# OATML-Markslab/ProteinGym

Measured on AMD Instinct MI355X. Metric: mutants scored/sec (ESM-1v 650M masked-marginal), higher is better.
Workload: dtype f16x3 (fp32 operands split into 2 fp16 planes, 3 fp16 MFMAs per product, fp32 accumulate)

## Files before the change

include/pgmi.h:

```cpp
#ifndef PGMI_H
#define PGMI_H

#include <stddef.h>
#include <stdint.h>

#ifdef __cplusplus
extern "C" {
#endif

#define PGMI_ABI_VERSION 5

#define PGMI_OK 0
#define PGMI_EINVAL (-1)
#define PGMI_ENOMEM (-2)
#define PGMI_EHIP (-3)
#define PGMI_ENODEV (-4)
#define PGMI_EPARSE (-5)
#define PGMI_EOVERFLOW (-6)

#define PGMI_ARCH_ESM1B 1
#define PGMI_ARCH_ESM2 2
#define PGMI_ARCH_TRANCEPTION 3
#define PGMI_ARCH_MSA 4
#define PGMI_ARCH_PROGEN2 5
// ... 111 lines not shown
int pgmi_op_gemm(int device, int precision, const float* A, const float* W, const float* bias,
                 const float* residual, int M, int N, int K, int epilogue ,
                 float* C);
int pgmi_op_qkln_prep(int device, const float* qkv, const float* q_w, const float* k_w, int B, int T, int H, int iters, float* qk,
                      float* v, double* ms);
int pgmi_op_attention(int device, int precision, const float* qkv, const int32_t* kv_len,
                      int B, int T, int H, int rotary, float* ctx);
int pgmi_op_causal_attention(int device, int lanes, const float* X, const float* W, const float* bias, int K, const float* qkv,
                             const float* conv, const float* rot_cos, const float* rot_sin, const float* slopes, int B, int T,
                             int heads, float* ctx);
int pgmi_op_prefix_attention(int device, const float* qkv, const int32_t* seg_off, int n_seg, const float* prefix_kv, int P, int heads,
                             int split, float* ctx);
int pgmi_op_cross_attention(int device, const float* q, const int32_t* seg_off, int n_seg, const float* mem_kv, int S, int heads,
                            int split, float* ctx);
int pgmi_op_rmsnorm(int device, const float* x, const float* w, int rows, int D, float eps, float* y);
int pgmi_op_geom_attention(int device, const float* proj, const float* rot, const float* trans, const int32_t* frame_mask,
                           int per_row_frames, const float* w_rot, const float* w_dist, int B, int S, int H, float* out);
int pgmi_op_geom_key_tile(int S);
int pgmi_op_moe(int device, const float* h, const float* gate, const float* w1, const float* w3, const float* w2, int M, int D, int F,
                int E, int top_k, int gated, float* out, int32_t* ids, float* weights);
int pgmi_op_tied_row_attention(int device, const float* qkv, int R, int C, int H, int splits, float* ctx, float* probs);
int pgmi_op_tied_row_splits(int R, int C, int H);
int pgmi_op_column_attention(int device, const float* X, const float* W, const float* bias, int K, int R, int C, int H, float* ctx);

int pgmi_tr_token_logprobs(pgmi_model* m, const int32_t* tokens, int B, int T, float* out);
int pgmi_tr_sequence_loglik(pgmi_model* m, const int32_t* tokens, const int32_t* lens, int B, int T,
                            const float* log_prior, int P, const int32_t* prior_a0, const int32_t* prior_row0,
                            const int32_t* prior_n, const int32_t* prior_flip, float alpha, float* out);
int pgmi_tr_sequence_loglik_shared(pgmi_model* m, const int32_t* tokens, const int32_t* ref, int B, int T,
                                   const float* log_prior, int P, const int32_t* prior_a0, const int32_t* prior_row0,
// ... 166 lines not shown
```

proteingym_amd/_lib.py:

```python
from __future__ import annotations

import ctypes as C
import os

import numpy as np

HERE = os.path.dirname(os.path.abspath(__file__))
LIB_PATH = os.path.join(HERE, "libpgmi.so")

ABI_VERSION = 5
ARCH_ESM1B, ARCH_ESM2, ARCH_TRANCEPTION = 1, 2, 3
ARCH_PROGEN2 = 5
ARCH_GPT = 6
ARCH_ESMC = 7
ARCH_SAPROT = 8
ARCH_POET = 9
ARCH_PROGEN3 = 10
ARCH_ESM3 = 11
ARCH_ESMIF1 = 12
GPT_POS_ROTARY, GPT_POS_LEARNED = 0, 1
PREC_FP32, PREC_BF16, PREC_F16X3 = 0, 1, 2
PRECISIONS = {"fp32": PREC_FP32, "bf16": PREC_BF16, "f16x3": PREC_F16X3}
K_NAMES = ["embed", "layernorm", "gemm_qkv", "attention", "gemm_out", "gemm_fc1", "gemm_fc2",
           "head", "score", "kept_rows", "moe_route", "geom", "cross_attention"]
# ... 119 lines not shown
    ("pgmi_unirep_destroy", None, [C.c_void_p]),
    ("pgmi_unirep_profile_model", C.c_void_p, [C.c_void_p]),
    ("pgmi_unirep_set_target", C.c_int, [C.c_void_p, _i32p, C.c_int]),
    ("pgmi_unirep_sequence_nll", C.c_int, [C.c_void_p, _i32p, _i64p, C.c_int64, C.c_int, _f64p, _i64p]),
    ("pgmi_unirep_token_logprobs", C.c_int, [C.c_void_p, _i32p, C.c_int, _f32p]),
    ("pgmi_op_mlstm_step", C.c_int, [C.c_void_p, _f32p, _f32p, _i32p, C.c_int, _f32p, _f32p, _f32p]),
    ("pgmi_bench_gemm", C.c_int, [C.c_int] * 9 + [_f64p]),
    ("pgmi_bench_gemm_ab", C.c_int, [C.c_int] * 7 + [_i32p, C.c_int, C.c_int, C.c_int, _f64p]),
    ("pgmi_op_attention", C.c_int, [C.c_int, C.c_int, _f32p, _i32p, C.c_int, C.c_int, C.c_int, C.c_int, _f32p]),
    ("pgmi_op_qkln_prep", C.c_int, [C.c_int, _f32p, _f32p, _f32p, C.c_int, C.c_int, C.c_int, C.c_int, _f32p, _f32p, _f64p]),
    ("pgmi_op_causal_attention", C.c_int, [C.c_int, C.c_int, _f32p, _f32p, _f32p, C.c_int, _f32p, _f32p, _f32p, _f32p, _f32p,
                                           C.c_int, C.c_int, C.c_int, _f32p]),
    ("pgmi_op_prefix_attention", C.c_int, [C.c_int, _f32p, _i32p, C.c_int, _f32p, C.c_int, C.c_int, C.c_int, _f32p]),
    ("pgmi_op_cross_attention", C.c_int, [C.c_int, _f32p, _i32p, C.c_int, _f32p, C.c_int, C.c_int, C.c_int, _f32p]),
    ("pgmi_op_rmsnorm", C.c_int, [C.c_int, _f32p, _f32p, C.c_int, C.c_int, C.c_float, _f32p]),
    ("pgmi_op_geom_attention", C.c_int, [C.c_int, _f32p, _f32p, _f32p, _i32p, C.c_int, _f32p, _f32p, C.c_int, C.c_int, C.c_int, _f32p]),
    ("pgmi_op_geom_key_tile", C.c_int, [C.c_int]),
    ("pgmi_op_moe", C.c_int, [C.c_int, _f32p, _f32p, _f32p, _f32p, _f32p, C.c_int, C.c_int, C.c_int, C.c_int, C.c_int, C.c_int, _f32p,
                              _i32p, _f32p]),
    ("pgmi_op_tied_row_attention", C.c_int, [C.c_int, _f32p, C.c_int, C.c_int, C.c_int, C.c_int, _f32p, _f32p]),
    ("pgmi_op_tied_row_splits", C.c_int, [C.c_int, C.c_int, C.c_int]),
    ("pgmi_op_column_attention", C.c_int, [C.c_int, _f32p, _f32p, _f32p, C.c_int, C.c_int, C.c_int, C.c_int, _f32p]),
    ("pgmi_msa_token_logprobs", C.c_int, [C.c_void_p, _i32p, C.c_int, C.c_int, _f32p]),
    ("pgmi_msa_masked_logprobs", C.c_int, [C.c_void_p, _i32p, C.c_int, C.c_int, C.c_int, _i32p, _i32p, C.c_int, _f32p]),
    ("pgmi_msa_cluster_counts", C.c_int, [C.c_int, C.POINTER(C.c_int8), C.c_int64, C.c_int64, C.c_int, C.c_double, _i32p, _f64p]),
    ("pgmi_msa_neighbor_counts", C.c_int, [C.c_int, C.POINTER(C.c_int8), C.c_int64, C.c_int64, C.c_int, C.c_double, _i32p, _f64p]),
]


def load():
# ... 68 lines not shown
```

proteingym_amd/csrc/api_esm.hip:

```cpp
#include "model.h"

namespace pgmi {

int create_esm(pgmi_model* m, const pgmi_config* cfg, const float* w, int64_t n_weights) {
    const size_t D = cfg->embed_dim, F = cfg->ffn_dim, V = cfg->vocab, dh = m->dh, Da = m->Da;
    BlobCursor c(m, w, n_weights);
    c.upload(&m->embed_tokens, V * D);
    if (cfg->arch == PGMI_ARCH_ESM1B) c.upload(&m->embed_positions, (size_t)(cfg->max_positions + 2) * D);
    if (cfg->emb_layer_norm_before) {
        c.upload(&m->lnb_w, D);
        c.upload(&m->lnb_b, D);
    }
    auto slot = [&](size_t col) -> size_t { return rotate_half_slot(col, dh); };
    const float qscale = 1.0f / sqrtf((float)dh);
    m->layers.resize(cfg->layers);
    std::vector<float> wq(3 * Da * D, 0.0f), bq(3 * Da, 0.0f), wo_r(D * Da, 0.0f);
    for (int l = 0; l < cfg->layers; ++l) {
        Layer& L = m->layers[l];
        c.upload(&L.ln1_w, D);
        c.upload(&L.ln1_b, D);
        pack_qkv_slots(c.take(3 * (D * D + D)), D, Da, slot, qscale, wq.data(), bq.data());
        c.linear(&L.wqkv, &L.wqkv16, wq.data(), wq.size(), D);
        c.upload(&L.bqkv, bq.data(), bq.size());
        pack_out_cols(c.take(D * D), D, Da, slot, wo_r.data());
// ... 21 lines not shown
    if ((!esm2_rotary(m->cfg.arch) && !esmc_blocks(m->cfg.arch)) || T <= m->rot_len) return PGMI_OK;
    return upload_rotate_half(m, std::max(T, 1026));
}

int upload_rotate_half(pgmi_model* m, int n) {
    const int rh = m->rot_halves;
    float inv[64];
    const int half = m->dh / 2;
    for (int i = 0; i < half; ++i) inv[i] = 1.0f / powf(10000.0f, (float)(2 * i) / (float)m->dh);
    return upload_rotary(m, n, rh, [&](int t, int g, int i) {
        const int j = (rh == 1) ? i : 32 * g + i;
        return j < half ? (float)t * inv[j] : 0.0f;
    });
}

int run_encoder(pgmi_model* m, int B, int T, const int32_t* keep, int n_keep, bool* compacted) {
    const pgmi_config& c = m->cfg;
    const int M = B * T, D = c.embed_dim, F = c.ffn_dim, N1 = m->fc1_cols, H = c.heads, Da = m->Da;
    hipStream_t s = m->stream;
    if (c.arch == PGMI_ARCH_ESM1B && T > c.max_positions) {
        set_error("Sequence length %d above maximum sequence length of %d", T, c.max_positions);
        return PGMI_EINVAL;
    }
    int rc = ensure_rotary(m, T);
    if (!rc) rc = reset_pad_keys(m, B, T);
    if (rc) return rc;
    {
        ProfScope p(m, PGMI_K_EMBED, 0, (double)M * D * 4);
        launch_seq_stats(m->tokens, B, T, m->embed_gather ? 0 : c.token_dropout, m->denom, m->pos_idx, m->kv_len, s, m->mask_id);
        if (c.arch == PGMI_ARCH_ESM3) { if ((rc = esm3_embed(m, B, T))) return rc; }
        else if (m->embed_gather) launch_gather_rows(m->embed_tokens, m->tokens, M, D, m->x, s);
        else launch_embed(m->tokens, m->denom, m->pos_idx, m->embed_tokens, m->embed_positions, c.token_dropout, M, T, D, m->x, s, m->mask_id);
        if (m->lnb_w) {
            launch_layernorm(m->x, m->lnb_w, m->lnb_b, M, D, 1e-5f, m->x, s);
            launch_zero_pad_rows(m->tokens, M, D, m->x, s);
        }
    }
    const double ln_bytes = 2.0 * M * D * 4;
    const int prec = c.precision;
    const int mode16 = (prec == PGMI_PREC_F16X3) ? 1 : 2;
    for (int l = 0; l < c.layers; ++l) {
        const Layer& L = m->layers[l];
        { ProfScope p(m, PGMI_K_LAYERNORM, 0, ln_bytes);
          if (prec == PGMI_PREC_FP32) launch_layernorm(m->x, L.ln1_w, L.ln1_b, M, D, 1e-5f, m->h, s);
          else launch_layernorm16(m->x, L.ln1_w, L.ln1_b, M, D, 1e-5f, m->h16, mode16, s); }
        const bool fused_qkv = prec != PGMI_PREC_FP32 && !L.q_ln;
        { ProfScope p(m, PGMI_K_GEMM_QKV, 2.0 * M * 3 * D * D, 0);
          if (fused_qkv) {
              GemmLaunch g = qkv_launch(m, L.wqkv16, L.bqkv, M, Da, D, T, m->Hs);
              g.bf = prec == PGMI_PREC_BF16;
              g.qkv.cos_t = m->rot_cos; g.qkv.sin_t = m->rot_sin; g.qkv.rotary = esm2_rotary(c.arch); g.qkv.rot_halves = m->rot_halves;
              rc = launch_gemm16(g);
          } else
              rc = linear(m, m->h, m->h16, L.wqkv, L.wqkv16, L.bqkv, nullptr, m->qkv, nullptr, M, 3 * Da, D, EPI_NONE);
          if (rc) return rc; }
        { ProfScope p(m, PGMI_K_ATTENTION, 4.0 * M * T * D, L.q_ln ? (double)M * D * 20 : 0);
          if (L.q_ln && (rc = launch_qkln_prep(m->qkv, L.q_ln, L.k_ln, 1e-5f, m->rot_cos, m->rot_sin, B, T, H, m->qk16, m->qk16_plane,
                                               m->vt16, m->vt16_plane, s)))
              return rc;
          const bool v2 = prec != PGMI_PREC_FP32;
          if (esm2_rotary(c.arch) && !v2) launch_rotary(m->qkv, m->rot_cos, m->rot_sin, M, T, m->Hs, s, m->rot_halves);
          if (v2) {
              AttLaunch a;
              a.qk16 = m->qk16, a.qk_plane = m->qk16_plane, a.vt16 = m->vt16, a.vt_plane = m->vt16_plane;
              a.B = B, a.T = T, a.H = H, a.head_dim = m->rot_halves * kHeadDim;
              a.kv_len = m->kv_len;
              a.out = prec == PGMI_PREC_F16X3 ? ATT_OUT_SPLIT : ATT_OUT_BF16;
              a.ctx16 = m->h16;
              a.stream = s;
              rc = launch_attention_f16x3_v2(a);
// ... 59 lines not shown
    const int prec = c.precision;
    const float* src = m->x;
    if (row_idx) {
        launch_gather_rows(m->x, row_idx, R, D, m->h, s);
        src = m->h;
    }
    if (prec == PGMI_PREC_FP32) launch_layernorm(src, m->lna_w, m->lna_b, R, D, 1e-5f, m->h, s);
    else launch_layernorm16(src, m->lna_w, m->lna_b, R, D, 1e-5f, m->h16, prec == PGMI_PREC_F16X3 ? 1 : 2, s);
    int rc = linear(m, m->h, m->h16, m->hd_w, m->hd16, m->hd_b, nullptr, m->g, nullptr, R, D, D, EPI_GELU);
    if (rc) return rc;
    launch_layernorm(m->g, m->hln_w, m->hln_b, R, D, 1e-5f, m->g, s);
    return PGMI_OK;
}


int run_rows(pgmi_model* m, int B, int T, int R, const int32_t* row_idx) {
    bool compacted = false;
    int rc = run_encoder(m, B, T, row_idx, R, &compacted);
    if (rc) return rc;
    return run_head(m, R, compacted ? nullptr : row_idx);
}

}

extern "C" {

int pgmi_token_logprobs(pgmi_model* m, const int32_t* tokens, int B, int T, float* out) {
    if (!m || !tokens || !out || B <= 0 || T <= 0) { set_error("bad argument"); return PGMI_EINVAL; }
    if (m->cfg.arch == PGMI_ARCH_SAPROT) { set_error("SaProt models are scored with pgmi_saprot_token_logprobs / pgmi_saprot_group_logprobs"); return PGMI_EINVAL; }
    if (T + 31 > m->max_rows) { set_error("T=%d exceeds workspace rows %d", T, m->max_rows); return PGMI_EINVAL; }
    int rc = check_tokens(tokens, B, T);
    if (rc) return rc;
    PGMI_HIP(hipSetDevice(m->device));
// ... 57 lines not shown
        mr[i] = positions[i] - s;
    }
    const int64_t n_sub = n_mut ? mut_off[n_mut] : 0;
    for (int64_t k = 0; k < n_sub; ++k)
        if (sub_pos[k] < 0 || sub_pos[k] >= n_tok || sub_wt[k] < 0 || sub_wt[k] >= PGMI_VOCAB || sub_mt[k] < 0 || sub_mt[k] >= PGMI_VOCAB) {
            set_error("substitution %lld out of range", (long long)k);
            return PGMI_EINVAL;
        }
    PGMI_HIP(hipSetDevice(m->device));
    pgmi_assay* a = new pgmi_assay();
    a->m = m; a->n_tok = n_tok; a->P = P; a->T = T; a->n_mut = n_mut; a->n_sub = n_sub;
    int rc = dev_upload(a->allocs, &a->wt, wt_tokens, (size_t)n_tok);
    if (!rc) rc = dev_upload(a->allocs, &a->positions, positions, (size_t)P);
    if (!rc) rc = dev_upload(a->allocs, &a->win_start, ws.data(), (size_t)P);
    if (!rc) rc = dev_upload(a->allocs, &a->mask_rel, mr.data(), (size_t)P);
    if (!rc) rc = dev_upload(a->allocs, &a->sub_pos, sub_pos, (size_t)n_sub);
    if (!rc) rc = dev_upload(a->allocs, &a->sub_wt, sub_wt, (size_t)n_sub);
    if (!rc) rc = dev_upload(a->allocs, &a->sub_mt, sub_mt, (size_t)n_sub);
    if (!rc) rc = dev_upload(a->allocs, &a->mut_off, mut_off, (size_t)(n_mut + 1));
    if (!rc) rc = dev_alloc(a->allocs, &a->table, (size_t)n_tok * PGMI_VOCAB);
    if (!rc) rc = dev_alloc(a->allocs, &a->scores, (size_t)n_mut);
    if (rc) { pgmi_assay_destroy(a); return rc; }
    m->assays.push_back(a);
    *out = a;
    return PGMI_OK;
}

void pgmi_assay_destroy(pgmi_assay* a) {
    if (!a) return;
    if (a->m) {
// ... 5 lines not shown
    for (void* p : a->allocs) hipFree(p);
    delete a;
}

int pgmi_assay_run(pgmi_model* m, pgmi_assay* a, double* scores_host, float* table_host, double* scores_dev) {
    if (!m || !a || a->m != m) { set_error("bad model/assay handle (assay belongs to another or a destroyed model)"); return PGMI_EINVAL; }
    PGMI_HIP(hipSetDevice(m->device));
    hipStream_t s = m->stream;
    const int T = a->T, V = m->cfg.vocab;
    const int per = rows_per_chunk(m, T);
    launch_fill_f32(a->table, (int64_t)a->n_tok * V, NAN, s);
    for (int p0 = 0; p0 < a->P; p0 += per) {
        const int bc = std::min(per, a->P - p0);
        launch_make_masked_windows(a->wt, a->win_start + p0, a->mask_rel + p0, bc, T, m->tokens, s);
        launch_row_index(a->mask_rel + p0, bc, T, m->row_idx, s);
        int rc = run_rows(m, bc, T, bc, m->row_idx);
        if (rc) return rc;
        launch_scatter_rows(m->lp, a->positions + p0, bc, V, a->table, s);
    }
    {
        ProfScope p(m, PGMI_K_SCORE, 0, (double)a->n_sub * 20);
        launch_score_mutants(a->table, V, a->sub_pos, a->sub_wt, a->sub_mt, a->mut_off, a->n_mut, a->scores, s);
    }
    PGMI_HIP(hipGetLastError());
    if (scores_dev && a->n_mut) PGMI_HIP(hipMemcpyAsync(scores_dev, a->scores, (size_t)a->n_mut * 8, hipMemcpyDeviceToDevice, s));
    if (scores_host && a->n_mut) PGMI_HIP(hipMemcpyAsync(scores_host, a->scores, (size_t)a->n_mut * 8, hipMemcpyDeviceToHost, s));
    if (table_host) PGMI_HIP(hipMemcpyAsync(table_host, a->table, (size_t)a->n_tok * V * 4, hipMemcpyDeviceToHost, s));
    PGMI_HIP(hipStreamSynchronize(s));
    return check_nonfinite(m);
}

int pgmi_pppl_create(pgmi_model* m, const uint8_t* tokens, const int64_t* seq_off, int64_t n_seq, pgmi_pppl** out) {
    if (!out) { set_error("null out"); return PGMI_EINVAL; }
    *out = nullptr;
    if (!m || !tokens || !seq_off || n_seq <= 0 || n_seq > 0x7fffffff) { set_error("bad argument"); return PGMI_EINVAL; }
    if (m->cfg.arch != PGMI_ARCH_ESM1B && m->cfg.arch != PGMI_ARCH_ESM2) { set_error("pseudo-ppl needs an ESM-1b/1v/ESM2 model"); return PGMI_EINVAL; }
    if (seq_off[0] != 0) { set_error("seq_off[0] must be 0"); return PGMI_EINVAL; }
    for (int64_t n = 0; n < n_seq; ++n) {
        const int64_t len = seq_off[n + 1] - seq_off[n];
        if (len < 2 || len > (1 << 24)) { set_error("sequence %lld has %lld tokens", (long long)n, (long long)len); return PGMI_EINVAL; }
        const uint8_t* t = tokens + seq_off[n];
        for (int64_t i = 0; i < len; ++i)
            if (t[i] >= PGMI_VOCAB || t[i] == PGMI_TOK_PAD) { set_error("token id %d invalid at sequence %lld, position %lld", (int)t[i], (long long)n, (long long)i); return PGMI_EINVAL; }
    }
// ... 115 lines not shown
```

proteingym_amd/csrc/api_model.hip:

```cpp
#include "model.h"

namespace pgmi {

static thread_local char g_err[1024] = "";
void set_error(const char* fmt, ...) {
    va_list ap;
    va_start(ap, fmt);
    vsnprintf(g_err, sizeof(g_err), fmt, ap);
    va_end(ap);
}

int prof_drain(pgmi_model* m) {
    if (m->events_used == 0) return PGMI_OK;
    PGMI_HIP(hipStreamSynchronize(m->stream));
    for (size_t i = 0; i < m->events_used; ++i) {
        float ms = 0.f;
        PGMI_HIP(hipEventElapsedTime(&ms, m->events[i].start, m->events[i].stop));
        m->prof_ms[m->events[i].cls] += ms;
    }
    m->events_used = 0;
    return PGMI_OK;
}

int check_cfg(const pgmi_config* c) {
    if (!c) { set_error("null config"); return PGMI_EINVAL; }
// ... 262 lines not shown
    int rc = PGMI_OK;
    auto alloc = [&](auto** p, size_t n) { if (!rc) rc = dev_alloc(m->allocs, p, n); };
    alloc(&m->x, R * D);
    alloc(&m->h, R * Dw);
    alloc(&m->qkv, R * 3 * Da);
    alloc(&m->g, R * (f32mode ? std::max(F, D) : D));
    if (!f32mode) {
        const size_t planes = c.precision == PGMI_PREC_F16X3 ? 2 : 1;
        m->h16_plane = R * Dw;
        m->g16_plane = R * F;
        alloc(&m->h16, m->h16_plane * planes);
        alloc(&m->g16, m->g16_plane * planes);
    }
    alloc(&m->nonfinite, (size_t)1);
    if (!f32mode) {
        m->qk16_plane = R * 2 * Da;
        m->vt16_plane = R * Da;
        alloc(&m->qk16, m->qk16_plane * 2);
        alloc(&m->vt16, m->vt16_plane * 2);
    }
    if (c.arch == PGMI_ARCH_MSA) {
        alloc(&m->xt, R * D);
        alloc(&m->msa_kv_len, (size_t)2048);
    }
    alloc(&m->lp, ((c.arch == PGMI_ARCH_GPT || c.arch == PGMI_ARCH_PROGEN3) && V > kWave ? (size_t)m->gpt_head_rows : R) * V);
    alloc(&m->denom, R);
    alloc(&m->tokens, R);
    alloc(&m->pos_idx, R);
    alloc(&m->kv_len, R);
    alloc(&m->row_idx, R);
    alloc(&m->aux_i, R);
    if (rc) return rc;
// ... 43 lines not shown
        case PGMI_ARCH_TRANCEPTION: rc = create_tranception(m, cfg, w, n_weights); break;
        case PGMI_ARCH_MSA: rc = create_msa(m, cfg, w, n_weights); break;
        case PGMI_ARCH_PROGEN2: rc = create_progen2(m, cfg, w, n_weights, arch_arg); break;
        case PGMI_ARCH_GPT: rc = create_gpt(m, cfg, w, n_weights, arch_arg); break;
        case PGMI_ARCH_ESMC: rc = create_esmc(m, cfg, w, n_weights); break;
        case PGMI_ARCH_SAPROT: rc = create_saprot(m, cfg, w, n_weights, arch_arg); break;
        case PGMI_ARCH_POET: rc = create_poet(m, cfg, w, n_weights, arch_arg); break;
        case PGMI_ARCH_PROGEN3: rc = create_progen3(m, cfg, w, n_weights, pg3); break;
        case PGMI_ARCH_ESM3: rc = create_esm3(m, cfg, w, n_weights, arch_arg); break;
        case PGMI_ARCH_ESMIF1: rc = create_esmif1(m, cfg, w, n_weights, arch_arg); break;
        default: rc = create_esm(m, cfg, w, n_weights);
    }
    if (!rc) rc = alloc_workspace(m);
    if (rc) { pgmi_model_destroy(m); return rc; }
    m->keep_rows = env_int("PGMI_KEEP_ROWS", 1);
    gemm_options_from_env();
    m->gemm_variant = env_int("PGMI_GEMM_VARIANT", 0);
    *out = m;
    return PGMI_OK;
}

}

extern "C" {

void pgmi_model_destroy(pgmi_model* m) {
    if (!m) return;
    hipSetDevice(m->device);
    if (m->stream) hipStreamSynchronize(m->stream);
    for (pgmi_assay* a : m->assays) {
// ... 7 lines not shown
        q->allocs.clear();
        q->m = nullptr;
    }
    m->pppls.clear();
    for (auto& e : m->events) { hipEventDestroy(e.start); hipEventDestroy(e.stop); }
    if (m->moe.counts_host) hipHostFree(m->moe.counts_host);
    for (void* p : m->allocs) hipFree(p);
    if (m->stream) hipStreamDestroy(m->stream);
    delete m;
}

int pgmi_model_device(const pgmi_model* m) { return m ? m->device : -1; }

int pgmi_set_option(const char* name, int64_t value) {
    if (!name) { set_error("null option name"); return PGMI_EINVAL; }
    int rc = gemm_set_option(name, (long long)value);
    if (rc) rc = att_set_option(name, (long long)value);
    if (rc) rc = eve_set_option(name, (long long)value);
    if (rc) rc = mpnn_set_option(name, (long long)value);
    if (rc) rc = unirep_set_option(name, (long long)value);
    if (rc) set_error("unknown option '%s' (gemm_half_tail, gemm_max_rows, att_xcd_local, att_v3, eve_max_rows, eve_fixed_sample, eve_prior_batch, mpnn_max_rows, unirep_max_rows)", name);
    return rc;
}

int pgmi_synchronize(pgmi_model* m) {
    if (!m) { set_error("null model"); return PGMI_EINVAL; }
    PGMI_HIP(hipStreamSynchronize(m->stream));
    return PGMI_OK;
}

int pgmi_profile_enable(pgmi_model* m, int on) {
    if (!m) { set_error("null model"); return PGMI_EINVAL; }
    int rc = prof_drain(m);
    m->prof = on != 0;
    return rc;
}
// ... 21 lines not shown
```

proteingym_amd/csrc/common.h:

```cpp
#pragma once
#include <hip/hip_runtime.h>
#include <stdint.h>
#include <stddef.h>

#include "../../include/pgmi.h"

namespace pgmi {

void set_error(const char* fmt, ...);

#define PGMI_HIP(expr)                                                                   \
    do {                                                                                 \
        hipError_t _e = (expr);                                                          \
        if (_e != hipSuccess) {                                                          \
            pgmi::set_error("%s failed: %s (%s:%d)", #expr, hipGetErrorString(_e),       \
                            __FILE__, __LINE__);                                         \
            return PGMI_EHIP;                                                            \
        }                                                                                \
    } while (0)

typedef float f32x4 __attribute__((ext_vector_type(4)));
typedef float f32x16 __attribute__((ext_vector_type(16)));

constexpr int kWave = 64;
// ... 44 lines not shown
void launch_embed(const int32_t* tokens, const float* scale, const int32_t* pos_idx,
                  const float* embed_tokens, const float* embed_positions, int token_dropout,
                  int rows, int T, int D, float* x, hipStream_t s, int mask_id = PGMI_TOK_MASK);
void launch_layernorm(const float* x, const float* w, const float* b, int rows, int D, float eps,
                      float* y, hipStream_t s);
void launch_gather_rows(const float* x, const int32_t* row_idx, int n, int D, float* y, hipStream_t s);
void launch_strided_index(int first, int stride, int n, int32_t* idx, hipStream_t s);
void launch_vocab_logsoftmax(const float* h, const float* E, const float* bias, int rows, int D,
                             int V, float* out, int32_t* nonfinite, hipStream_t s);
void launch_layernorm16(const float* x, const float* w, const float* b, int rows, int D, float eps,
                        unsigned short* y16, int mode, hipStream_t s);
int launch_rmsnorm16(const float* x, const float* w, int rows, int D, float eps, unsigned short* y16, hipStream_t s);
void launch_scatter_rows(const float* src, const int32_t* dst_row, int n, int V, float* table,
                         hipStream_t s);
void launch_row_index(const int32_t* mask_rel, int B, int T, int32_t* out, hipStream_t s);
void launch_fill_f32(float* p, int64_t n, float v, hipStream_t s);
void launch_seq_loglik(const float* lp, const int32_t* tokens, const int32_t* lens, int B, int T, int V,
                       const float* prior, const int32_t* a0, const int32_t* row0, const int32_t* n,
                       const int32_t* flip, float alpha, const float* eve, float beta, int eve_fallback, float* out, hipStream_t s);
void launch_seq_loglik_ragged(const float* lp, const int32_t* tokens, const int32_t* seq_off, const int32_t* seq_p,
                              const int32_t* seq_root, int B, int T, int V, const float* prior, const int32_t* a0,
                              const int32_t* row0, const int32_t* n, const int32_t* flip, float alpha, const float* eve, float beta,
                              int eve_fallback, float* out, hipStream_t s);
void launch_pg2_seq_loglik(const float* lp, const int32_t* col, const int32_t* n_kept, int B, int T, int V, float* out, hipStream_t s);
void launch_embed_learned(const int32_t* tokens, const float* E, const float* P, int rows, int T, int D, float* x, hipStream_t s);
void launch_embed_scaled_pos(const int32_t* tokens, const int32_t* pos, const float* E, const float* P, float scale, int rows, int D,
                             float* x, hipStream_t s);
void launch_wide_logsoftmax(const float* logits, int ldl, int rows, int V, const int32_t* tgt, float* out, int32_t* nonfinite,
                            hipStream_t s);
void launch_seq_sum(const float* terms, const int32_t* off, int B, double* out, hipStream_t s);
// ... 254 lines not shown
```

proteingym_amd/csrc/elementwise.hip:

```cpp
#include "common.h"

namespace pgmi {

__device__ __forceinline__ float wave_sum(float v) {
#pragma unroll
    for (int o = 32; o > 0; o >>= 1) v += __shfl_xor(v, o);
    return v;
}
__device__ __forceinline__ float wave_max(float v) {
#pragma unroll
    for (int o = 32; o > 0; o >>= 1) v = fmaxf(v, __shfl_xor(v, o));
    return v;
}
__device__ __forceinline__ double wave_sum_d(double v) {
#pragma unroll
    for (int o = 32; o > 0; o >>= 1) v += __shfl_xor(v, o);
    return v;
}
__device__ __forceinline__ int wave_sum_i(int v) {
#pragma unroll
    for (int o = 32; o > 0; o >>= 1) v += __shfl_xor(v, o);
    return v;
}

// ... 314 lines not shown
    const int rI = i / V, c = i % V;
    table[(size_t)dst_row[rI] * V + c] = src[i];
}
void launch_scatter_rows(const float* src, const int32_t* dst_row, int n, int V, float* table, hipStream_t s) {
    hipLaunchKernelGGL(scatter_rows_kernel, dim3((n * V + 255) / 256), dim3(256), 0, s, src, dst_row, n, V, table);
}

__global__ void row_index_kernel(const int32_t* __restrict__ mask_rel, int B, int T, int32_t* __restrict__ out) {
    const int b = blockIdx.x * blockDim.x + threadIdx.x;
    if (b < B) out[b] = b * T + mask_rel[b];
}
void launch_row_index(const int32_t* mask_rel, int B, int T, int32_t* out, hipStream_t s) {
    hipLaunchKernelGGL(row_index_kernel, dim3((B + 255) / 256), dim3(256), 0, s, mask_rel, B, T, out);
}

__global__ void fill_f32_kernel(float* p, int64_t n, float v) {
    const int64_t i = (int64_t)blockIdx.x * blockDim.x + threadIdx.x;
    if (i < n) p[i] = v;
}
void launch_fill_f32(float* p, int64_t n, float v, hipStream_t s) {
    hipLaunchKernelGGL(fill_f32_kernel, dim3((unsigned)((n + 255) / 256)), dim3(256), 0, s, p, n, v);
}

__global__ __launch_bounds__(256) void vocab_logsoftmax_kernel(const float* __restrict__ h,
                                                               const float* __restrict__ E,
                                                               const float* __restrict__ bias, int rows,
                                                               int D, int V, float* __restrict__ out,
                                                               int32_t* __restrict__ nonfinite) {
    const int row = blockIdx.x * 4 + (threadIdx.x >> 6);
    const int lane = threadIdx.x & 63;
// ... 431 lines not shown
```

proteingym_amd/csrc/model.h:

```cpp
#pragma once
#include <math.h>
#include <stdlib.h>
#include <cmath>
#include <algorithm>
#include <stdarg.h>
#include <stdio.h>
#include <string.h>

#include <string>
#include <vector>

#include "common.h"
#include "gemm16x_kernel.h"

namespace pgmi {

struct W16 {
    unsigned short* p = nullptr;
    float out_scale = 1.0f;
};

struct Layer {
    float *ln1_w, *ln1_b, *wqkv, *bqkv, *wo, *bo, *ln2_w, *ln2_b, *w1, *b1, *w2, *b2;
    W16 wqkv16, wo16, w116, w216;
// ... 74 lines not shown
    int32_t* poet_meta = nullptr;
    int if1_enc = 0, if1_pos_len = 0;
    float *if1_mem = nullptr, *if1_pos = nullptr;
    unsigned short* if1_mem16 = nullptr;
    int e3_vheads = 0, e3_Kp = 0;
    float *e3_struct_embed = nullptr, *e3_const = nullptr;
    int32_t *e3_stok = nullptr, *e3_plddt = nullptr, *e3_mask = nullptr;
    float *e3_rot = nullptr, *e3_trans = nullptr;
    size_t e3_cap = 0;
    int e3_T = 0;
    bool e3_framed = false;
    unsigned short *h16 = nullptr, *g16 = nullptr;
    size_t h16_plane = 0, g16_plane = 0;
    unsigned short *qk16 = nullptr, *vt16 = nullptr;
    size_t qk16_plane = 0, vt16_plane = 0;
    int32_t* nonfinite = nullptr;
    int gemm_variant = 0;
    int keep_rows = 1;
    int last_B = 0, last_T = 0;
    int dh = kHeadDim;
    int rot_halves = 1;
    int Hs = 0;
    int Da = 0;
    float *rot_cos = nullptr, *rot_sin = nullptr;
    int rot_len = 0;
    float* zeros = nullptr;
    int max_rows = 0;
    float *x = nullptr, *h = nullptr, *qkv = nullptr, *g = nullptr, *lp = nullptr, *denom = nullptr;
    int32_t *tokens = nullptr, *pos_idx = nullptr, *kv_len = nullptr, *row_idx = nullptr, *aux_i = nullptr;
    bool prof = false;
    std::vector<ProfEvent> events;
    size_t events_used = 0;
    double prof_ms[PGMI_K_COUNT] = {0};
    int64_t prof_n[PGMI_K_COUNT] = {0};
    double prof_flops[PGMI_K_COUNT] = {0};
    double prof_bytes[PGMI_K_COUNT] = {0};
};

struct pgmi_assay {
    pgmi_model* m = nullptr;
    int n_tok = 0, P = 0, T = 0;
    int64_t n_mut = 0, n_sub = 0;
    std::vector<void*> allocs;
    int32_t *wt = nullptr, *positions = nullptr, *win_start = nullptr, *mask_rel = nullptr;
    int32_t *sub_pos = nullptr, *sub_wt = nullptr, *sub_mt = nullptr;
    int64_t* mut_off = nullptr;
    float* table = nullptr;
    double* scores = nullptr;
};

struct pgmi_pppl {
    pgmi_model* m = nullptr;
    int64_t N = 0;
    std::vector<int64_t> off;
    std::vector<void*> allocs;
    uint8_t* tok8 = nullptr;
    int64_t* off_dev = nullptr;
    int64_t last_rows = 0, last_chunks = 0, last_tokens = 0, last_padded = 0;
};
// ... 59 lines not shown
int check_cfg(const pgmi_config* c);
int check_tokens(const int32_t* tokens, int B, int T, int n_ids = PGMI_VOCAB);
int check_vocab(const int32_t* tokens, int B, int T, int V);
int env_int(const char* name, int dflt);
int make_w16(std::vector<void*>& pool, const float* host, size_t n, size_t K, int precision, hipStream_t s, W16* out);
int linear(pgmi_model* m, const float* in32, const unsigned short* in16, const float* W32, const W16& w16, const float* bias,
           const float* residual, float* out32, unsigned short* out16, int M, int N, int K, int epi);
GemmLaunch qkv_launch(pgmi_model* m, const W16& w16, const float* bias, int M, int Da, int K, int T, int H);
int check_nonfinite(pgmi_model* m);
int reset_pad_keys(pgmi_model* m, int B, int T);
int model_create(const pgmi_config* cfg, const float* w, int64_t n_weights, int device, pgmi_model** out, int arch_arg,
                 const pgmi_pg3_params* pg3 = nullptr);
int create_esm(pgmi_model* m, const pgmi_config* cfg, const float* w, int64_t n_weights);
int ensure_rotary(pgmi_model* m, int T);
int upload_rotate_half(pgmi_model* m, int n);
int run_encoder(pgmi_model* m, int B, int T, const int32_t* keep = nullptr, int n_keep = 0, bool* compacted = nullptr);
int head_hidden(pgmi_model* m, int R, const int32_t* row_idx);
int run_head(pgmi_model* m, int R, const int32_t* row_idx);
int run_rows(pgmi_model* m, int B, int T, int R, const int32_t* row_idx);
int create_tranception(pgmi_model* m, const pgmi_config* cfg, const float* w, int64_t n_weights);
int create_progen2(pgmi_model* m, const pgmi_config* cfg, const float* w, int64_t n_weights, int rotary_dim);
int create_gpt(pgmi_model* m, const pgmi_config* cfg, const float* w, int64_t n_weights, int pos_kind);
int64_t gpt_weight_count(const pgmi_config* c, int pos_kind);
int decoder_check(pgmi_model* m, int arch, int T);
int run_decoder(pgmi_model* m, int B, int T, const AttRagged* rg = nullptr, int rows = 0, double att_flops = 0);
int narrow_head(pgmi_model* m, int M);
int decoder_token_logprobs(pgmi_model* m, int arch, const int32_t* tokens, int B, int T, float* out);
int decoder_sequence_loglik(pgmi_model* m, int arch, const int32_t* tokens, const int32_t* lens, int B, int T, double* sum, int32_t* n_targets);
int pg3_check(const pgmi_config* c, const pgmi_pg3_params* p);
int64_t pg3_weight_count(const pgmi_config* c, const pgmi_pg3_params* p);
int create_progen3(pgmi_model* m, const pgmi_config* cfg, const float* w, int64_t n_weights, const pgmi_pg3_params* p);
void pack_swiglu(const float* w1, const float* w3, size_t F, size_t D, float* dst);
int moe_ws_alloc(std::vector<void*>& pool, pgmi_model::MoeWs* ws, size_t rows, size_t layers, int D, int F, int E, int top_k, int gated);
int dense_ffn(pgmi_model* m, const pgmi_model::MoeWs& ws, const W16& w1, const W16& w2, const unsigned short* h16, unsigned short* g16,
// ... 128 lines not shown
```

Measured before the change: 18090.

## Share layer-0 QKV across masked windows and broadcast Q/K/V planes

When every masked-marginal window in a chunk covers the same wild-type span, layer 0 runs layernorm and the fused QKV GEMM on only 2T rows: the unmasked sequence and one row per masked position. A new kernel then broadcasts those Q/K and V^T fp16 planes to all B sequences, patching in the masked token's row. This removes about B*T rows of layer-0 QKV GEMM work per chunk, at the cost of a gather, a broadcast copy, and extra plane memory (share_rows). Later layers diverge and still run in full.

```diff
diff --git a/include/pgmi.h b/include/pgmi.h
--- a/include/pgmi.h
+++ b/include/pgmi.h
@@ -149,6 +149,8 @@
 int pgmi_op_cross_attention(int device, const float* q, const int32_t* seg_off, int n_seg, const float* mem_kv, int S, int heads,
                             int split, float* ctx);
 int pgmi_op_rmsnorm(int device, const float* x, const float* w, int rows, int D, float eps, float* y);
+int pgmi_op_broadcast_qkv_planes(int device, const uint16_t* src_qk, const uint16_t* src_vt, const int32_t* mask_rel, int B, int T,
+                                 int Da, uint16_t* qk, uint16_t* vt);
 int pgmi_op_geom_attention(int device, const float* proj, const float* rot, const float* trans, const int32_t* frame_mask,
                            int per_row_frames, const float* w_rot, const float* w_dist, int B, int S, int H, float* out);
 int pgmi_op_geom_key_tile(int S);
diff --git a/proteingym_amd/_lib.py b/proteingym_amd/_lib.py
--- a/proteingym_amd/_lib.py
+++ b/proteingym_amd/_lib.py
@@ -157,6 +157,8 @@
     ("pgmi_op_prefix_attention", C.c_int, [C.c_int, _f32p, _i32p, C.c_int, _f32p, C.c_int, C.c_int, C.c_int, _f32p]),
     ("pgmi_op_cross_attention", C.c_int, [C.c_int, _f32p, _i32p, C.c_int, _f32p, C.c_int, C.c_int, C.c_int, _f32p]),
     ("pgmi_op_rmsnorm", C.c_int, [C.c_int, _f32p, _f32p, C.c_int, C.c_int, C.c_float, _f32p]),
+    ("pgmi_op_broadcast_qkv_planes", C.c_int, [C.c_int, C.POINTER(C.c_uint16), C.POINTER(C.c_uint16), _i32p, C.c_int, C.c_int, C.c_int,
+                                               C.POINTER(C.c_uint16), C.POINTER(C.c_uint16)]),
     ("pgmi_op_geom_attention", C.c_int, [C.c_int, _f32p, _f32p, _f32p, _i32p, C.c_int, _f32p, _f32p, C.c_int, C.c_int, C.c_int, _f32p]),
     ("pgmi_op_geom_key_tile", C.c_int, [C.c_int]),
     ("pgmi_op_moe", C.c_int, [C.c_int, _f32p, _f32p, _f32p, _f32p, _f32p, C.c_int, C.c_int, C.c_int, C.c_int, C.c_int, C.c_int, _f32p,
diff --git a/proteingym_amd/csrc/api_esm.hip b/proteingym_amd/csrc/api_esm.hip
--- a/proteingym_amd/csrc/api_esm.hip
+++ b/proteingym_amd/csrc/api_esm.hip
@@ -59,7 +59,7 @@
     });
 }
 
-int run_encoder(pgmi_model* m, int B, int T, const int32_t* keep, int n_keep, bool* compacted) {
+int run_encoder(pgmi_model* m, int B, int T, const int32_t* keep, int n_keep, bool* compacted, const ShareL0* share) {
     const pgmi_config& c = m->cfg;
     const int M = B * T, D = c.embed_dim, F = c.ffn_dim, N1 = m->fc1_cols, H = c.heads, Da = m->Da;
     hipStream_t s = m->stream;
@@ -84,21 +84,43 @@
     const double ln_bytes = 2.0 * M * D * 4;
     const int prec = c.precision;
     const int mode16 = (prec == PGMI_PREC_F16X3) ? 1 : 2;
+    const int Tp = (T + 31) / 32 * 32;
+    const int share_opt = share_layer0_option();
+    const bool share0 = share && 2 * Tp <= m->share_rows && (share_opt >= 0 ? share_opt : m->share_layer0) != 0;
     for (int l = 0; l < c.layers; ++l) {
         const Layer& L = m->layers[l];
-        { ProfScope p(m, PGMI_K_LAYERNORM, 0, ln_bytes);
-          if (prec == PGMI_PREC_FP32) launch_layernorm(m->x, L.ln1_w, L.ln1_b, M, D, 1e-5f, m->h, s);
-          else launch_layernorm16(m->x, L.ln1_w, L.ln1_b, M, D, 1e-5f, m->h16, mode16, s); }
         const bool fused_qkv = prec != PGMI_PREC_FP32 && !L.q_ln;
-        { ProfScope p(m, PGMI_K_GEMM_QKV, 2.0 * M * 3 * D * D, 0);
+        const bool shared = l == 0 && share0 && fused_qkv;
+        const int Mq = shared ? 2 * T : M;
+        { ProfScope p(m, PGMI_K_LAYERNORM, 0, shared ? 4.0 * Mq * D * 4 : ln_bytes);
+          const float* xin = m->x;
+          if (shared) {
+              launch_gather_rows(m->x, share->rows, Mq, D, m->qkv, s);
+              xin = m->qkv;
+          }
+          if (prec == PGMI_PREC_FP32) launch_layernorm(xin, L.ln1_w, L.ln1_b, Mq, D, 1e-5f, m->h, s);
+          else launch_layernorm16(xin, L.ln1_w, L.ln1_b, Mq, D, 1e-5f, m->h16, mode16, s); }
+        unsigned short* const share_qk = shared ? m->qk16 + (size_t)m->max_rows * 2 * Da : nullptr;
+        unsigned short* const share_vt = shared ? m->vt16 + (size_t)m->max_rows * Da : nullptr;
+        { ProfScope p(m, PGMI_K_GEMM_QKV, 2.0 * Mq * 3 * D * D, 0);
           if (fused_qkv) {
-              GemmLaunch g = qkv_launch(m, L.wqkv16, L.bqkv, M, Da, D, T, m->Hs);
+              GemmLaunch g = qkv_launch(m, L.wqkv16, L.bqkv, Mq, Da, D, T, m->Hs);
+              if (shared) g.out16 = share_qk, g.qkv.vt16 = share_vt;
               g.bf = prec == PGMI_PREC_BF16;
               g.qkv.cos_t = m->rot_cos; g.qkv.sin_t = m->rot_sin; g.qkv.rotary = esm2_rotary(c.arch); g.qkv.rot_halves = m->rot_halves;
               rc = launch_gemm16(g);
           } else
               rc = linear(m, m->h, m->h16, L.wqkv, L.wqkv16, L.bqkv, nullptr, m->qkv, nullptr, M, 3 * Da, D, EPI_NONE);
           if (rc) return rc; }
+        if (shared) {
+            ProfScope p(m, PGMI_K_ATTENTION, 0, 2.0 * B * (2.0 * T * 2 * Da + 2.0 * Da * Tp) * 2);
+            BroadcastQkv bq;
+            bq.src_qk = share_qk, bq.src_vt = share_vt, bq.qk16 = m->qk16, bq.vt16 = m->vt16;
+            bq.qk_plane = m->qk16_plane, bq.vt_plane = m->vt16_plane;
+            bq.src_rows = (size_t)m->share_rows, bq.dst_rows = (size_t)m->max_rows;
+            bq.mask_rel = share->mask_rel, bq.B = B, bq.T = T, bq.Da = Da, bq.stream = s;
+            if ((rc = launch_broadcast_qkv_planes(bq))) return rc;
+        }
         { ProfScope p(m, PGMI_K_ATTENTION, 4.0 * M * T * D, L.q_ln ? (double)M * D * 20 : 0);
           if (L.q_ln && (rc = launch_qkln_prep(m->qkv, L.q_ln, L.k_ln, 1e-5f, m->rot_cos, m->rot_sin, B, T, H, m->qk16, m->qk16_plane,
                                                m->vt16, m->vt16_plane, s)))
@@ -188,9 +210,9 @@
 }
 
 
-int run_rows(pgmi_model* m, int B, int T, int R, const int32_t* row_idx) {
+int run_rows(pgmi_model* m, int B, int T, int R, const int32_t* row_idx, const ShareL0* share) {
     bool compacted = false;
-    int rc = run_encoder(m, B, T, row_idx, R, &compacted);
+    int rc = run_encoder(m, B, T, row_idx, R, &compacted, share);
     if (rc) return rc;
     return run_head(m, R, compacted ? nullptr : row_idx);
 }
@@ -278,6 +300,26 @@
     if (!rc) rc = dev_upload(a->allocs, &a->positions, positions, (size_t)P);
     if (!rc) rc = dev_upload(a->allocs, &a->win_start, ws.data(), (size_t)P);
     if (!rc) rc = dev_upload(a->allocs, &a->mask_rel, mr.data(), (size_t)P);
+    bool one_window = P > 0 && m->share_rows > 0 && 2 * ((T + 31) / 32 * 32) <= m->share_rows;
+    for (int i = 0; one_window && i < P; ++i) one_window = ws[i] == ws[0];
+    for (int i = 0; one_window && i < T; ++i) one_window = wt_tokens[ws[0] + i] != m->mask_id;
+    if (!rc && one_window) {
+        const int per = rows_per_chunk(m, T);
+        std::vector<int32_t> src((size_t)((P + per - 1) / per) * 2 * T);
+        for (int p0 = 0; p0 < P; p0 += per) {
+            const int bc = std::min(per, P - p0);
+            int32_t* r = &src[(size_t)(p0 / per) * 2 * T];
+            for (int t = 0; t < T; ++t) {
+                int b = 0;
+                while (b < bc - 1 && mr[p0 + b] == t) ++b;
+                r[t] = b * T + t;
+                r[T + t] = t;
+            }
+            for (int b = 0; b < bc; ++b) r[T + mr[p0 + b]] = b * T + mr[p0 + b];
+        }
+        a->share_per = per;
+        rc = dev_upload(a->allocs, &a->share_src, src.data(), src.size());
+    }
     if (!rc) rc = dev_upload(a->allocs, &a->sub_pos, sub_pos, (size_t)n_sub);
     if (!rc) rc = dev_upload(a->allocs, &a->sub_wt, sub_wt, (size_t)n_sub);
     if (!rc) rc = dev_upload(a->allocs, &a->sub_mt, sub_mt, (size_t)n_sub);
@@ -313,7 +355,9 @@
         const int bc = std::min(per, a->P - p0);
         launch_make_masked_windows(a->wt, a->win_start + p0, a->mask_rel + p0, bc, T, m->tokens, s);
         launch_row_index(a->mask_rel + p0, bc, T, m->row_idx, s);
-        int rc = run_rows(m, bc, T, bc, m->row_idx);
+        const bool one_window = a->share_src && per == a->share_per;
+        const ShareL0 sh{a->mask_rel + p0, one_window ? a->share_src + (size_t)(p0 / per) * 2 * T : nullptr};
+        int rc = run_rows(m, bc, T, bc, m->row_idx, one_window ? &sh : nullptr);
         if (rc) return rc;
         launch_scatter_rows(m->lp, a->positions + p0, bc, V, a->table, s);
     }
@@ -327,6 +371,51 @@
     if (table_host) PGMI_HIP(hipMemcpyAsync(table_host, a->table, (size_t)a->n_tok * V * 4, hipMemcpyDeviceToHost, s));
     PGMI_HIP(hipStreamSynchronize(s));
     return check_nonfinite(m);
+}
+
+int pgmi_op_broadcast_qkv_planes(int device, const uint16_t* src_qk, const uint16_t* src_vt, const int32_t* mask_rel, int B, int T, int Da,
+                                 uint16_t* qk, uint16_t* vt) {
+    if (!src_qk || !src_vt || !mask_rel || !qk || !vt) { set_error("bad argument"); return PGMI_EINVAL; }
+    BroadcastQkv c;
+    c.B = B, c.T = T, c.Da = Da;
+    const size_t Tp = T > 0 ? ((size_t)T + 31) / 32 * 32 : 0;
+    c.src_rows = 2 * Tp, c.dst_rows = (size_t)std::max(B, 0) * Tp;
+    c.qk_plane = (c.dst_rows + c.src_rows) * 2 * (size_t)std::max(Da, 0), c.vt_plane = c.qk_plane / 2;
+    int rc = broadcast_qkv_check(c, false);
+    if (rc) return rc;
+    for (int b = 0; b < B; ++b)
+        if (mask_rel[b] < 0 || mask_rel[b] >= T) { set_error("mask_rel[%d]=%d out of range", b, mask_rel[b]); return PGMI_EINVAL; }
+    if (pgmi_device_count() <= 0) { set_error("no HIP device visible"); return PGMI_ENODEV; }
+    PGMI_HIP(hipSetDevice(device));
+    std::vector<void*> pool;
+    auto cleanup = [&]() { for (void* p : pool) hipFree(p); };
+    unsigned short *dqk = nullptr, *dvt = nullptr;
+    int32_t* dmask = nullptr;
+    if ((rc = dev_alloc(pool, &dqk, 2 * c.qk_plane)) || (rc = dev_alloc(pool, &dvt, 2 * c.vt_plane)) ||
+        (rc = dev_upload(pool, &dmask, mask_rel, (size_t)B))) {
+        cleanup();
+        return rc;
+    }
+    const size_t sq = (size_t)2 * T * 2 * Da, sv = 2 * (size_t)Da * Tp;
+    const size_t nq = (size_t)B * T * 2 * Da, nv = (size_t)B * Da * Tp;
+    unsigned short *const sqk = dqk + c.dst_rows * 2 * Da, *const svt = dvt + c.dst_rows * Da;
+    c.qk16 = dqk, c.vt16 = dvt, c.src_qk = sqk, c.src_vt = svt, c.mask_rel = dmask;
+    hipError_t e = hipMemset(dqk, 0xFF, 2 * c.qk_plane * 2);
+    if (e == hipSuccess) e = hipMemset(dvt, 0xFF, 2 * c.vt_plane * 2);
+    for (int p = 0; p < 2 && e == hipSuccess; ++p) {
+        e = hipMemcpy(sqk + p * c.qk_plane, src_qk + p * sq, sq * 2, hipMemcpyHostToDevice);
+        if (e == hipSuccess) e = hipMemcpy(svt + p * c.vt_plane, src_vt + p * sv, sv * 2, hipMemcpyHostToDevice);
+    }
+    if (e == hipSuccess) rc = launch_broadcast_qkv_planes(c);
+    if (e == hipSuccess) e = hipDeviceSynchronize();
+    for (int p = 0; p < 2 && !rc && e == hipSuccess; ++p) {
+        e = hipMemcpy(qk + p * nq, dqk + p * c.qk_plane, nq * 2, hipMemcpyDeviceToHost);
+        if (e == hipSuccess) e = hipMemcpy(vt + p * nv, dvt + p * c.vt_plane, nv * 2, hipMemcpyDeviceToHost);
+    }
+    cleanup();
+    if (rc) return rc;
+    if (e != hipSuccess) { set_error("broadcast_qkv_planes op failed: %s", hipGetErrorString(e)); return PGMI_EHIP; }
+    return PGMI_OK;
 }
 
 int pgmi_pppl_create(pgmi_model* m, const uint8_t* tokens, const int64_t* seq_off, int64_t n_seq, pgmi_pppl** out) {
diff --git a/proteingym_amd/csrc/api_model.hip b/proteingym_amd/csrc/api_model.hip
--- a/proteingym_amd/csrc/api_model.hip
+++ b/proteingym_amd/csrc/api_model.hip
@@ -9,6 +9,9 @@
     vsnprintf(g_err, sizeof(g_err), fmt, ap);
     va_end(ap);
 }
+
+static int g_share_layer0 = -1;
+int share_layer0_option() { return g_share_layer0; }
 
 int prof_drain(pgmi_model* m) {
     if (m->events_used == 0) return PGMI_OK;
@@ -301,8 +304,9 @@
     }
     alloc(&m->nonfinite, (size_t)1);
     if (!f32mode) {
-        m->qk16_plane = R * 2 * Da;
-        m->vt16_plane = R * Da;
+        if (c.arch == PGMI_ARCH_ESM1B || c.arch == PGMI_ARCH_ESM2) m->share_rows = 2048;
+        m->qk16_plane = (R + m->share_rows) * 2 * Da;
+        m->vt16_plane = (R + m->share_rows) * Da;
         alloc(&m->qk16, m->qk16_plane * 2);
         alloc(&m->vt16, m->vt16_plane * 2);
     }
@@ -376,6 +380,7 @@
     if (!rc) rc = alloc_workspace(m);
     if (rc) { pgmi_model_destroy(m); return rc; }
     m->keep_rows = env_int("PGMI_KEEP_ROWS", 1);
+    m->share_layer0 = env_int("PGMI_SHARE_LAYER0", 1);
     gemm_options_from_env();
     m->gemm_variant = env_int("PGMI_GEMM_VARIANT", 0);
     *out = m;
@@ -413,12 +418,17 @@
 
 int pgmi_set_option(const char* name, int64_t value) {
     if (!name) { set_error("null option name"); return PGMI_EINVAL; }
+    if (!strcmp(name, "share_layer0")) {
+        if (value < -1 || value > 1) { set_error("share_layer0: %lld is not 0, 1 or -1", (long long)value); return PGMI_EINVAL; }
+        g_share_layer0 = (int)value;
+        return PGMI_OK;
+    }
     int rc = gemm_set_option(name, (long long)value);
     if (rc) rc = att_set_option(name, (long long)value);
     if (rc) rc = eve_set_option(name, (long long)value);
     if (rc) rc = mpnn_set_option(name, (long long)value);
     if (rc) rc = unirep_set_option(name, (long long)value);
-    if (rc) set_error("unknown option '%s' (gemm_half_tail, gemm_max_rows, att_xcd_local, att_v3, eve_max_rows, eve_fixed_sample, eve_prior_batch, mpnn_max_rows, unirep_max_rows)", name);
+    if (rc) set_error("unknown option '%s' (share_layer0, gemm_half_tail, gemm_max_rows, att_xcd_local, att_v3, eve_max_rows, eve_fixed_sample, eve_prior_batch, mpnn_max_rows, unirep_max_rows)", name);
     return rc;
 }
 
diff --git a/proteingym_amd/csrc/common.h b/proteingym_amd/csrc/common.h
--- a/proteingym_amd/csrc/common.h
+++ b/proteingym_amd/csrc/common.h
@@ -82,6 +82,23 @@
 void launch_scatter_rows(const float* src, const int32_t* dst_row, int n, int V, float* table,
                          hipStream_t s);
 void launch_row_index(const int32_t* mask_rel, int B, int T, int32_t* out, hipStream_t s);
+__host__ __device__ __forceinline__ int vt_key_pos(int t) {
+    const int tk = t & 31;
+    return (t & ~31) + ((tk & 0x13) | ((tk & 4) << 1) | ((tk & 8) >> 1));
+}
+struct BroadcastQkv {
+    const unsigned short* src_qk = nullptr;
+    const unsigned short* src_vt = nullptr;
+    unsigned short* qk16 = nullptr;
+    unsigned short* vt16 = nullptr;
+    size_t qk_plane = 0, vt_plane = 0;
+    size_t src_rows = 0, dst_rows = 0;
+    const int32_t* mask_rel = nullptr;
+    int B = 0, T = 0, Da = 0;
+    hipStream_t stream = nullptr;
+};
+int broadcast_qkv_check(const BroadcastQkv& c, bool pointers = true);
+int launch_broadcast_qkv_planes(const BroadcastQkv& c);
 void launch_fill_f32(float* p, int64_t n, float v, hipStream_t s);
 void launch_seq_loglik(const float* lp, const int32_t* tokens, const int32_t* lens, int B, int T, int V,
                        const float* prior, const int32_t* a0, const int32_t* row0, const int32_t* n,
diff --git a/proteingym_amd/csrc/elementwise.hip b/proteingym_amd/csrc/elementwise.hip
--- a/proteingym_amd/csrc/elementwise.hip
+++ b/proteingym_amd/csrc/elementwise.hip
@@ -352,6 +352,87 @@
     hipLaunchKernelGGL(row_index_kernel, dim3((B + 255) / 256), dim3(256), 0, s, mask_rel, B, T, out);
 }
 
+typedef unsigned short u16x8 __attribute__((ext_vector_type(8)));
+constexpr int kBcastUnit = 1024;
+__global__ __launch_bounds__(256) void broadcast_qkv_planes_kernel(const u16x8* __restrict__ src_qk, const u16x8* __restrict__ src_vt,
+                                                                   u16x8* __restrict__ qk, u16x8* __restrict__ vt, size_t qk_plane8,
+                                                                   size_t vt_plane8, const int32_t* __restrict__ mask_rel, int B, int T,
+                                                                   int Tp, int Da, int units_per_seq, long long n_units) {
+    const int Cq = Da / 4, Cv = Tp / 8;
+    const int nq1 = T * Cq, nv1 = Da * Cv;
+    const int per_seq = 2 * (nq1 + nv1);
+    for (long long u = blockIdx.x; u < n_units; u += gridDim.x) {
+        const int b = (int)(u / units_per_seq);
+        if (b >= B) return;
+        const int s = (int)(u - (long long)b * units_per_seq);
+        int mk = mask_rel[b];
+        if (mk < 0 || mk >= T) mk = -1;
+        const int kp = mk < 0 ? -1 : vt_key_pos(mk);
+        u16x8 v[4];
+        u16x8* dst[4];
+#pragma unroll
+        for (int k = 0; k < 4; ++k) {
+            const int i = s * kBcastUnit + k * 256 + (int)threadIdx.x;
+            dst[k] = nullptr;
+            if (i >= per_seq) continue;
+            if (i < 2 * nq1) {
+                const int p = i >= nq1, j = i - p * nq1, t = j / Cq, c = j - t * Cq;
+                const size_t base = (size_t)p * qk_plane8 + (size_t)c;
+                v[k] = src_qk[base + (size_t)(t == mk ? T + t : t) * Cq];
+                dst[k] = qk + base + ((size_t)b * T + t) * Cq;
+            } else {
+                const int i2 = i - 2 * nq1, p = i2 >= nv1, j = i2 - p * nv1, r = j / Cv, cc = j - r * Cv;
+                const size_t base = (size_t)p * vt_plane8 + (size_t)cc;
+                u16x8 w = src_vt[base + (size_t)r * Cv];
+                if (kp >= 0 && cc == (kp >> 3)) w[kp & 7] = src_vt[base + ((size_t)Da + r) * Cv][kp & 7];
+                v[k] = w;
+                dst[k] = vt + base + ((size_t)b * Da + r) * Cv;
+            }
+        }
+#pragma unroll
+        for (int k = 0; k < 4; ++k)
+            if (dst[k]) *dst[k] = v[k];
+    }
+}
+
+int broadcast_qkv_check(const BroadcastQkv& c, bool pointers) {
+    auto misaligned = [](const void* p) { return ((uintptr_t)p & 15) != 0; };
+    if (pointers && (!c.src_qk || !c.src_vt || !c.qk16 || !c.vt16 || !c.mask_rel)) { set_error("broadcast_qkv_planes: null pointer"); return PGMI_EINVAL; }
+    if (c.B <= 0 || c.T <= 0 || c.Da <= 0 || c.Da % kHeadDim) {
+        set_error("broadcast_qkv_planes: unsupported shape B=%d T=%d Da=%d", c.B, c.T, c.Da);
+        return PGMI_EINVAL;
+    }
+    if ((pointers && (misaligned(c.src_qk) || misaligned(c.src_vt) || misaligned(c.qk16) || misaligned(c.vt16))) || c.qk_plane % 8 || c.vt_plane % 8) {
+        set_error("broadcast_qkv_planes: planes must be 16-byte aligned");
+        return PGMI_EINVAL;
+    }
+    const size_t Tp = ((size_t)c.T + 31) / 32 * 32, Da = (size_t)c.Da;
+    if (2 * Tp > c.src_rows || (size_t)c.B * Tp > c.dst_rows || c.dst_rows * 2 * Da > c.qk_plane || c.dst_rows * Da > c.vt_plane) {
+        set_error("broadcast_qkv_planes: B=%d sequences of T=%d tokens do not fit planes of %zu source / %zu destination rows", c.B, c.T,
+                  c.src_rows, c.dst_rows);
+        return PGMI_EINVAL;
+    }
+    if (2 * ((size_t)c.T * (Da / 4) + Da * (Tp / 8)) > (size_t)0x7fffffff - kBcastUnit) {
+        set_error("broadcast_qkv_planes: T=%d x Da=%d exceeds the 32-bit chunk index", c.T, c.Da);
+        return PGMI_EINVAL;
+    }
+    return PGMI_OK;
+}
+
+int launch_broadcast_qkv_planes(const BroadcastQkv& c) {
+    const int rc = broadcast_qkv_check(c, true);
+    if (rc) return rc;
+    const int Tp = (c.T + 31) / 32 * 32;
+    const long long per_seq = 2ll * ((long long)c.T * (c.Da / 4) + (long long)c.Da * (Tp / 8));
+    const int units_per_seq = (int)((per_seq + kBcastUnit - 1) / kBcastUnit);
+    const long long n_units = (long long)c.B * units_per_seq;
+    hipLaunchKernelGGL(broadcast_qkv_planes_kernel, dim3((unsigned)(n_units < 2048 ? n_units : 2048)), dim3(256), 0, c.stream,
+                       reinterpret_cast<const u16x8*>(c.src_qk), reinterpret_cast<const u16x8*>(c.src_vt), reinterpret_cast<u16x8*>(c.qk16),
+                       reinterpret_cast<u16x8*>(c.vt16), c.qk_plane / 8, c.vt_plane / 8, c.mask_rel, c.B, c.T, Tp, c.Da, units_per_seq, n_units);
+    PGMI_HIP(hipGetLastError());
+    return PGMI_OK;
+}
+
 __global__ void fill_f32_kernel(float* p, int64_t n, float v) {
     const int64_t i = (int64_t)blockIdx.x * blockDim.x + threadIdx.x;
     if (i < n) p[i] = v;
diff --git a/proteingym_amd/csrc/model.h b/proteingym_amd/csrc/model.h
--- a/proteingym_amd/csrc/model.h
+++ b/proteingym_amd/csrc/model.h
@@ -112,6 +112,7 @@
     size_t h16_plane = 0, g16_plane = 0;
     unsigned short *qk16 = nullptr, *vt16 = nullptr;
     size_t qk16_plane = 0, vt16_plane = 0;
+    int share_rows = 0, share_layer0 = 1;
     int32_t* nonfinite = nullptr;
     int gemm_variant = 0;
     int keep_rows = 1;
@@ -141,6 +142,8 @@
     int64_t n_mut = 0, n_sub = 0;
     std::vector<void*> allocs;
     int32_t *wt = nullptr, *positions = nullptr, *win_start = nullptr, *mask_rel = nullptr;
+    int32_t* share_src = nullptr;
+    int share_per = 0;
     int32_t *sub_pos = nullptr, *sub_wt = nullptr, *sub_mt = nullptr;
     int64_t* mut_off = nullptr;
     float* table = nullptr;
@@ -230,10 +233,16 @@
 int create_esm(pgmi_model* m, const pgmi_config* cfg, const float* w, int64_t n_weights);
 int ensure_rotary(pgmi_model* m, int T);
 int upload_rotate_half(pgmi_model* m, int n);
-int run_encoder(pgmi_model* m, int B, int T, const int32_t* keep = nullptr, int n_keep = 0, bool* compacted = nullptr);
+struct ShareL0 {
+    const int32_t* mask_rel;
+    const int32_t* rows;
+};
+int run_encoder(pgmi_model* m, int B, int T, const int32_t* keep = nullptr, int n_keep = 0, bool* compacted = nullptr,
+                const ShareL0* share = nullptr);
 int head_hidden(pgmi_model* m, int R, const int32_t* row_idx);
 int run_head(pgmi_model* m, int R, const int32_t* row_idx);
-int run_rows(pgmi_model* m, int B, int T, int R, const int32_t* row_idx);
+int run_rows(pgmi_model* m, int B, int T, int R, const int32_t* row_idx, const ShareL0* share = nullptr);
+int share_layer0_option();
 int create_tranception(pgmi_model* m, const pgmi_config* cfg, const float* w, int64_t n_weights);
 int create_progen2(pgmi_model* m, const pgmi_config* cfg, const float* w, int64_t n_weights, int rotary_dim);
 int create_gpt(pgmi_model* m, const pgmi_config* cfg, const float* w, int64_t n_weights, int pos_kind);
```

Measured after the change: 18200 (median of 6 runs). No clear change (+0.6%).
